# piotrkawa/audio-deepfake-adversarial-attacks

Measured on AMD Instinct MI355X. Metric: adversarial utterances/sec, PGD-40 LCNN+LFCC 4s@16kHz, higher is better.
Workload: dtype f32

## Files before the change

audio_deepfake_adversarial_attacks_amd/csrc/lfcc_stft.hip:

```cpp

#include <hip/hip_runtime.h>
#include <math.h>
#include <stdint.h>
#include <stdlib.h>

#include "advstep_frontend.h"
#include "advstep_common.h"

namespace {

constexpr int kN = 256;
constexpr int kNfft = 2 * kN;
constexpr int kBins = kN + 1;
constexpr int kWavesPerBlock = 4;
constexpr int kThreads = kWavesPerBlock * 64;
constexpr int kFramesPerBlockBwd = 4;

__device__ __forceinline__ float2 cmul(float2 a, float2 b) { return make_float2(a.x * b.x - a.y * b.y, a.x * b.y + a.y * b.x); }
__device__ __forceinline__ float2 cadd(float2 a, float2 b) { return make_float2(a.x + b.x, a.y + b.y); }
__device__ __forceinline__ float2 csub(float2 a, float2 b) { return make_float2(a.x - b.x, a.y - b.y); }
__device__ __forceinline__ float2 conjf2(float2 a) { return make_float2(a.x, -a.y); }

__device__ __forceinline__ void wave_lds_sync() {
    __builtin_amdgcn_fence(__ATOMIC_RELEASE, "workgroup");
    __builtin_amdgcn_wave_barrier();
    __builtin_amdgcn_fence(__ATOMIC_ACQUIRE, "workgroup");
}

#include "stft_tables.inc"

__device__ __forceinline__ float2 cmulf(float2 a, float2 b) {
    return make_float2(fmaf(a.x, b.x, -(a.y * b.y)), fmaf(a.x, b.y, a.y * b.x));
}
__device__ __forceinline__ float2 cmulc(float2 a, float cr, float ci) { return cmulf(a, make_float2(cr, ci)); }

template <bool INV>
__device__ __forceinline__ void fft4(float2 &a, float2 &b, float2 &c, float2 &d) {
    const float2 s02 = cadd(a, c), d02 = csub(a, c), s13 = cadd(b, d), d13 = csub(b, d);
    const float2 r = INV ? make_float2(-d13.y, d13.x) : make_float2(d13.y, -d13.x);
    a = cadd(s02, s13);
    b = cadd(d02, r);
    c = csub(s02, s13);
    d = csub(d02, r);
}

template <bool INV>
__device__ __forceinline__ void fft16(float2 (&x)[16]) {
    constexpr float C1 = 0.92387953251128674f, S1 = 0.38268343236508977f, H = 0.70710678118654752f;
#pragma unroll
    for (int n2 = 0; n2 < 4; ++n2) fft4<INV>(x[n2], x[4 + n2], x[8 + n2], x[12 + n2]);
    const float sg = INV ? 1.0f : -1.0f;
    x[4 + 1] = cmulc(x[4 + 1], C1, sg * S1);
    x[8 + 1] = cmulc(x[8 + 1], H, sg * H);
    x[12 + 1] = cmulc(x[12 + 1], S1, sg * C1);
    x[4 + 2] = cmulc(x[4 + 2], H, sg * H);
    x[8 + 2] = INV ? make_float2(-x[8 + 2].y, x[8 + 2].x) : make_float2(x[8 + 2].y, -x[8 + 2].x);
    x[12 + 2] = cmulc(x[12 + 2], -H, sg * H);
    x[4 + 3] = cmulc(x[4 + 3], S1, sg * C1);
    x[8 + 3] = cmulc(x[8 + 3], -H, sg * H);
    x[12 + 3] = cmulc(x[12 + 3], -C1, -sg * S1);
#pragma unroll
    for (int k1 = 0; k1 < 4; ++k1) fft4<INV>(x[4 * k1], x[4 * k1 + 1], x[4 * k1 + 2], x[4 * k1 + 3]);
#pragma unroll
    for (int i = 0; i < 4; ++i)
#pragma unroll
        for (int j = i + 1; j < 4; ++j) {
            const float2 t = x[4 * i + j];
            x[4 * i + j] = x[4 * j + i];
            x[4 * j + i] = t;
        }
}

__device__ __forceinline__ int here(int v) {
    asm volatile("" : "+v"(v));
    return v;
}

__device__ __forceinline__ void phase_done(float2 (&x)[16]) {
    asm volatile("" : "+v"(x[0].x), "+v"(x[0].y), "+v"(x[1].x), "+v"(x[1].y), "+v"(x[2].x), "+v"(x[2].y), "+v"(x[3].x), "+v"(x[3].y),
                      "+v"(x[4].x), "+v"(x[4].y), "+v"(x[5].x), "+v"(x[5].y), "+v"(x[6].x), "+v"(x[6].y), "+v"(x[7].x), "+v"(x[7].y)
                 :: "memory");
    asm volatile("" : "+v"(x[8].x), "+v"(x[8].y), "+v"(x[9].x), "+v"(x[9].y), "+v"(x[10].x), "+v"(x[10].y), "+v"(x[11].x), "+v"(x[11].y),
                      "+v"(x[12].x), "+v"(x[12].y), "+v"(x[13].x), "+v"(x[13].y), "+v"(x[14].x), "+v"(x[14].y), "+v"(x[15].x), "+v"(x[15].y)
                 :: "memory");
}

template <int BASE>
__device__ __forceinline__ void half_done(float2 (&x)[16]) {
    asm volatile("" : "+v"(x[BASE].x), "+v"(x[BASE].y), "+v"(x[BASE + 1].x), "+v"(x[BASE + 1].y), "+v"(x[BASE + 2].x), "+v"(x[BASE + 2].y),
                      "+v"(x[BASE + 3].x), "+v"(x[BASE + 3].y), "+v"(x[BASE + 4].x), "+v"(x[BASE + 4].y), "+v"(x[BASE + 5].x),
                      "+v"(x[BASE + 5].y), "+v"(x[BASE + 6].x), "+v"(x[BASE + 6].y), "+v"(x[BASE + 7].x), "+v"(x[BASE + 7].y)
                 :: "memory");
}

constexpr int kPitch = 17;
constexpr int kFrameSlots = 16 * kPitch;
constexpr int kGroup = 4;

__device__ __forceinline__ void lds_wave_fence() { asm volatile("s_waitcnt lgkmcnt(0)" ::: "memory"); }

template <bool INV>
__device__ __forceinline__ void fft256_reg(float2 (&x)[16], const float2 *twl, float2 *blk, int l) {
    fft16<INV>(x);
    phase_done(x);
#pragma unroll
    for (int j = 1; j < 16; ++j) {
        const float2 t = twl[l * kPitch + j];
        x[j] = cmulf(x[j], INV ? conjf2(t) : t);
    }
    lds_wave_fence();
#pragma unroll
    for (int j = 0; j < 16; ++j) blk[j * kPitch + l] = x[j];
    lds_wave_fence();
#pragma unroll
    for (int j = 0; j < 16; ++j) x[j] = blk[l * kPitch + j];
    fft16<INV>(x);
}

__device__ __forceinline__ int P(int i) { return i ^ (((i >> 4) & 3) * 5); }
constexpr int kNPad = kN + kN / 16;
constexpr int kStageTw = 3 * (4 + 16 + 64);

template <bool INV>
__device__ __forceinline__ void fft256(float2 *a, float2 *b, const float2 *__restrict__ tw, int lane) {
#pragma unroll
    for (int stage = 0; stage < 4; ++stage) {
        const int Ns = 1 << (2 * stage);
        const int k = lane & (Ns - 1);
        float2 v0 = a[P(lane)], v1 = a[P(lane + 64)], v2 = a[P(lane + 128)], v3 = a[P(lane + 192)];
        if (stage > 0) {
            const float2 *ts = tw + (stage == 1 ? 0 : (stage == 2 ? 12 : 60));
            float2 w1 = ts[k], w2 = ts[Ns + k], w3 = ts[2 * Ns + k];
            if (INV) w1 = conjf2(w1), w2 = conjf2(w2), w3 = conjf2(w3);
            v1 = cmul(v1, w1), v2 = cmul(v2, w2), v3 = cmul(v3, w3);
        }
        const float2 s02 = cadd(v0, v2), d02 = csub(v0, v2), s13 = cadd(v1, v3), d13 = csub(v1, v3);
        const float2 r = INV ? make_float2(-d13.y, d13.x) : make_float2(d13.y, -d13.x);
        const int j0 = ((lane - k) << 2) + k;
        b[P(j0)] = cadd(s02, s13);
        b[P(j0 + Ns)] = cadd(d02, r);
        b[P(j0 + 2 * Ns)] = csub(s02, s13);
        b[P(j0 + 3 * Ns)] = csub(d02, r);
        wave_lds_sync();
        float2 *t = a;
        a = b;
        b = t;
    }
}

__device__ __forceinline__ void load_frame(const float *__restrict__ xb, const float *__restrict__ w, int T, int f,
                                           int hop, float2 *z, int lane) {
    const int q_first = f * hop - kN;
    if (q_first >= 0 && q_first + kNfft <= T && ((q_first & 1) == 0) && ((reinterpret_cast<uintptr_t>(xb) & 7u) == 0)) {
        const float2 *x2 = reinterpret_cast<const float2 *>(xb + q_first);
        const float2 *w2 = reinterpret_cast<const float2 *>(w);
#pragma unroll
        for (int i = 0; i < 4; ++i) {
            const int n = lane + 64 * i;
            const float2 xv = x2[n], wv = w2[n];
            z[P(n)] = make_float2(wv.x * xv.x, wv.y * xv.y);
        }
        return;
    }
#pragma unroll
    for (int i = 0; i < 4; ++i) {
        const int n = lane + 64 * i;
        int q0 = f * hop + 2 * n - kN, q1 = q0 + 1;
        q0 = q0 < 0 ? -q0 : q0;
        q0 = q0 >= T ? 2 * (T - 1) - q0 : q0;
        q1 = q1 < 0 ? -q1 : q1;
        q1 = q1 >= T ? 2 * (T - 1) - q1 : q1;
        z[P(n)] = make_float2(w[2 * n] * xb[q0], w[2 * n + 1] * xb[q1]);
    }
}

__device__ __forceinline__ void unpack_real(const float2 *Z, const float2 *__restrict__ tw512, float2 *xs, int lane) {
    for (int k = lane; k < kN; k += 64) {
        const float2 zk = Z[P(k)], zc = conjf2(Z[P((kN - k) & (kN - 1))]);
        const float2 e = make_float2(0.5f * (zk.x + zc.x), 0.5f * (zk.y + zc.y));
        const float2 d = make_float2(0.5f * (zk.x - zc.x), 0.5f * (zk.y - zc.y));
        const float2 o = cmul(tw512[k], make_float2(d.y, -d.x));
        xs[k] = cadd(e, o);
    }
    if (lane == 0) xs[kN] = make_float2(Z[P(0)].x - Z[P(0)].y, 0.0f);
}

struct Lds {
    float2 a[kWavesPerBlock][kNPad];
    float2 b[kWavesPerBlock][kNPad];
    __device__ __forceinline__ float2 *xs_of(int wave) { return b[wave]; }
    __device__ __forceinline__ const float2 *xs_of(int wave) const { return b[wave]; }
    float2 tw[kStageTw];
    float2 tw512[kN];
    float red[kWavesPerBlock];
};

__device__ __forceinline__ float2 stage_twiddle(int m) {
    const int stage = m < 12 ? 1 : (m < 60 ? 2 : 3), base = stage == 1 ? 0 : (stage == 2 ? 12 : 60), Ns = 1 << (2 * stage);
    const int t = (m - base) / Ns + 1, k = (m - base) % Ns;
    return kTw256[(t * k * (64 / Ns)) & 255];
}

__device__ __forceinline__ void fill_twiddles(Lds &L) {
    for (int m = threadIdx.x; m < kN; m += kThreads) {
        if (m < kStageTw) L.tw[m] = stage_twiddle(m);
        L.tw512[m] = kTw512[m];
    }
}

constexpr int kFramesPerBlockFwd = 16;

__global__ __launch_bounds__(kThreads) void stft_bands_kernel(const float *__restrict__ x, const float *__restrict__ w,
                                                              const int32_t *__restrict__ fb_start,
                                                              const float *__restrict__ fb_w, int span,
                                                              float *__restrict__ band_db, float *__restrict__ bmax, int T,
                                                              int NF, int hop, int M) {
    __shared__ Lds L;
    fill_twiddles(L);
    __syncthreads();
    const int wave = threadIdx.x >> 6, lane = threadIdx.x & 63;
    const int64_t b = blockIdx.y;
    float vmax = -INFINITY;
    for (int r = 0; r < kFramesPerBlockFwd / kWavesPerBlock; ++r) {
        const int f = blockIdx.x * kFramesPerBlockFwd + r * kWavesPerBlock + wave;
        if (f >= NF) break;
        load_frame(x + b * T, w, T, f, hop, L.a[wave], lane);
        wave_lds_sync();
        fft256<false>(L.a[wave], L.b[wave], L.tw, lane);
        unpack_real(L.a[wave], L.tw512, L.xs_of(wave), lane);
        wave_lds_sync();
        float *row = band_db + (b * NF + f) * M;
        for (int m = lane; m < M; m += 64) {
            const int f0 = fb_start[m];
            float band = 0.0f;
            for (int j = 0; j < span; ++j) {
                const int k = f0 + j;
                if (k < kBins) {
                    const float2 z = L.xs_of(wave)[k];
                    band = fmaf(fb_w[m * span + j], fmaf(z.x, z.x, z.y * z.y), band);
                }
            }
            const float db = 3.010299956639812f * __log2f(band > kAmin ? band : (band != band ? band : kAmin));
            row[m] = db;
            vmax = max_nan(vmax, db);
        }
        wave_lds_sync();
    }
    vmax = wave_reduce(vmax, MaxNanOp());
    if (lane == 0) L.red[wave] = vmax;
    __syncthreads();
    if (threadIdx.x == 0) {
        float r = L.red[0];
        for (int i = 1; i < kWavesPerBlock; ++i) r = max_nan(r, L.red[i]);
        bmax[b * gridDim.x + blockIdx.x] = r;
    }
}

constexpr int kMaxSpanT = 8, kMaxBands = 128;

__device__ __forceinline__ void frame_spectrum(const float *__restrict__ xb, const float *__restrict__ w, int T, int f,
                                               int hop, Lds &L, int wave, int lane) {
    load_frame(xb, w, T, f, hop, L.a[wave], lane);
    wave_lds_sync();
    fft256<false>(L.a[wave], L.b[wave], L.tw, lane);
    unpack_real(L.a[wave], L.tw512, L.xs_of(wave), lane);
    wave_lds_sync();
}

__device__ __forceinline__ float2 one_sided_scale(float2 gk, int k) {
    if (k == 0 || k == kN) gk.y = 0.0f;
    else gk.x *= 0.5f, gk.y *= 0.5f;
    return gk;
}

template <bool PRESCALED>
__device__ __forceinline__ void spectrum_grad_to_frame(Lds &L, int wave, int lane, const float *__restrict__ w, float *dst,
                                                       bool live) {
    if (!PRESCALED) {
        for (int k = lane; k < kBins; k += 64) L.xs_of(wave)[k] = one_sided_scale(L.xs_of(wave)[k], k);
        wave_lds_sync();
    }
    for (int k = lane; k < kN; k += 64) {
        const float2 gk = L.xs_of(wave)[k], gc = conjf2(L.xs_of(wave)[kN - k]);
        const float2 e = cadd(gk, gc), d = csub(gk, gc);
        const float2 wd = cmul(conjf2(L.tw512[k]), d);
        L.a[wave][P(k)] = make_float2(e.x - wd.y, e.y + wd.x);
    }
    wave_lds_sync();
    fft256<true>(L.a[wave], L.b[wave], L.tw, lane);
    for (int n = lane; n < kN; n += 64) {
        const float2 z = L.a[wave][P(n)];
        const float2 wv = reinterpret_cast<const float2 *>(w)[n];
        reinterpret_cast<float2 *>(dst)[n] = live ? make_float2(wv.x * z.x, wv.y * z.y) : make_float2(0.0f, 0.0f);
    }
    wave_lds_sync();
}

template <int STRIDE>
__device__ __attribute__((noinline)) void overlap_add_frames_cold(const float *dframe, float *__restrict__ dxb, int f_base, int NF, int hop,
                                                                  int T, int tid, int nthreads);

template <int STRIDE>
__device__ __forceinline__ void overlap_add_frames(const float *dframe, float *__restrict__ dxb, int f_base, int NF, int hop, int T,
                                                   int tid, int nthreads) {
    const int p_lo = f_base * hop;
    const int frames_here = (NF - f_base) < kFramesPerBlockBwd ? (NF - f_base) : kFramesPerBlockBwd;
    const int p_hi = p_lo + (frames_here - 1) * hop + kNfft;
    auto add_from = [&](int p, float &acc) {
        if (p < p_lo || p >= p_hi) return;
#pragma unroll
        for (int fl = 0; fl < kFramesPerBlockBwd; ++fl) {
            const int n = p - p_lo - fl * hop;
            if (fl < frames_here && n >= 0 && n < kNfft) acc += dframe[fl * STRIDE + n];
        }
    };
    const bool near_left = p_lo < 2 * kN, near_right = p_hi > T;
    const int t_first = p_lo - kN, span_all = p_hi - p_lo;
    for (int i = tid; i < span_all; i += nthreads) {
        const int t = t_first + i;
        if (t < 0 || t >= T) continue;
        float acc = 0.0f;
        add_from(t + kN, acc);
        if (near_left && t >= 1 && t <= kN) add_from(kN - t, acc);
        if (near_right && t <= T - 2 && t >= T - 1 - kN) add_from(2 * (T - 1) - t + kN, acc);
        if (acc != 0.0f) atomicAdd(dxb + t, acc);
    }
    if (!(near_left || near_right)) return;
    for (int i = tid; i < span_all; i += nthreads) {
        const int p = p_lo + i, q = p - kN;
        int t = -1;
        if (q < 0) t = -q;
        else if (q >= T) t = 2 * (T - 1) - q;
        if (t < 0 || t >= T) continue;
        const int pd = t + kN;
        if (pd >= p_lo && pd < p_hi) continue;
        float acc = 0.0f;
        add_from(p, acc);
        if (acc != 0.0f) atomicAdd(dxb + t, acc);
    }
}

__device__ __forceinline__ void overlap_add_block(const float (*dframe)[kNfft], float *__restrict__ dxb, int f_base, int NF,
                                                  int hop, int T) {
    overlap_add_frames<kNfft>(&dframe[0][0], dxb, f_base, NF, hop, T, threadIdx.x, kThreads);
}

template <int STRIDE>
__device__ __attribute__((noinline)) void overlap_add_frames_cold(const float *dframe, float *__restrict__ dxb, int f_base, int NF, int hop,
                                                                  int T, int tid, int nthreads) {
    overlap_add_frames<STRIDE>(dframe, dxb, f_base, NF, hop, T, tid, nthreads);
}

template <int SPAN_CAP>
struct LdsBwd {
    Lds c;
    float dframe[kFramesPerBlockBwd][kNfft];
    float fbt_w[kBins * SPAN_CAP];
    int32_t fbt_start[kBins];
    float drow[kWavesPerBlock][kMaxBands];
};

template <int SPAN_CAP>
__global__ __launch_bounds__(kThreads) void stft_bands_backward_kernel(const float *__restrict__ x,
                                                                       const float *__restrict__ w,
                                                                       const float *__restrict__ dband,
                                                                       const int32_t *__restrict__ fbt_start,
                                                                       const float *__restrict__ fbt_w, int span_t,
                                                                       float *__restrict__ dx, int T, int NF, int hop,
                                                                       int M) {
    extern __shared__ __attribute__((aligned(16))) unsigned char raw[];
    LdsBwd<SPAN_CAP> &S = *reinterpret_cast<LdsBwd<SPAN_CAP> *>(raw);
    Lds &L = S.c;
    {
        static_assert(kN == kThreads, "one twiddle pair per thread");
        constexpr int kWIt = (kBins * SPAN_CAP + kThreads - 1) / kThreads;
        const int m = threadIdx.x, nw = kBins * span_t;
        const float2 t0 = stage_twiddle(m < kStageTw ? m : 0), t1 = kTw512[m];
        const int32_t s0 = fbt_start[m], s1 = fbt_start[kThreads + (m < kBins - kThreads ? m : 0)];
        float wq[kWIt];
#pragma unroll
        for (int j = 0; j < kWIt; ++j) {
            const int i = m + j * kThreads;
            wq[j] = fbt_w[i < nw ? i : nw - 1];
        }
        if (m < kStageTw) L.tw[m] = t0;
        L.tw512[m] = t1;
        S.fbt_start[m] = s0;
        if (m < kBins - kThreads) S.fbt_start[kThreads + m] = s1;
#pragma unroll
        for (int j = 0; j < kWIt; ++j) {
            const int i = m + j * kThreads;
            if (i < nw) S.fbt_w[i] = wq[j];
        }
    }
    __syncthreads();
    const int wave = threadIdx.x >> 6, lane = threadIdx.x & 63;
    const int64_t b = blockIdx.y;
    const int f_base = blockIdx.x * kFramesPerBlockBwd;
    const float *xb = x + b * T;
    for (int r = 0; r < kFramesPerBlockBwd / kWavesPerBlock; ++r) {
        const int fl = r * kWavesPerBlock + wave;
        const int f = f_base + fl;
        const bool live = f < NF;
        const float *drow_g = dband + (b * NF + (live ? f : NF - 1)) * M;
        for (int m = lane; m < M; m += 64) S.drow[wave][m] = drow_g[m];
        load_frame(xb, w, T, live ? f : NF - 1, hop, L.a[wave], lane);
        wave_lds_sync();
        fft256<false>(L.a[wave], L.b[wave], L.tw, lane);
        const float *drow = S.drow[wave];
        auto grad_of_bin = [&](int k, float2 xk) {
            const int m0 = S.fbt_start[k];
            float dp = 0.0f;
            for (int j = 0; j < span_t; ++j) {
                const int m = m0 + j;
                if (m < M) dp = fmaf(S.fbt_w[k * span_t + j], drow[m], dp);
            }
            return one_sided_scale(make_float2(2.0f * xk.x * dp, 2.0f * xk.y * dp), k);
        };
        {
            const float2 *Z = L.a[wave];
            for (int k = lane; k < kN; k += 64) {
                const float2 zk = Z[P(k)], zc = conjf2(Z[P((kN - k) & (kN - 1))]);
                const float2 e = make_float2(0.5f * (zk.x + zc.x), 0.5f * (zk.y + zc.y));
                const float2 d = make_float2(0.5f * (zk.x - zc.x), 0.5f * (zk.y - zc.y));
                const float2 o = cmul(L.tw512[k], make_float2(d.y, -d.x));
                L.xs_of(wave)[k] = grad_of_bin(k, cadd(e, o));
            }
            if (lane == 0) L.xs_of(wave)[kN] = grad_of_bin(kN, make_float2(Z[P(0)].x - Z[P(0)].y, 0.0f));
        }
        wave_lds_sync();
        spectrum_grad_to_frame<true>(L, wave, lane, w, S.dframe[fl], live);
    }
    __syncthreads();
    overlap_add_block(S.dframe, dx + b * T, f_base, NF, hop, T);
}

#ifndef STFT_FWD_GROUPS
#define STFT_FWD_GROUPS 2
#endif
constexpr int kGroupsPerWave = STFT_FWD_GROUPS;
constexpr int kBandsFramesPerBlock = kWavesPerBlock * kGroupsPerWave * kGroup;

struct LdsReg {
    float2 blk[kWavesPerBlock][kGroup][kFrameSlots];
    float2 twl[16 * kPitch];
    float red[kWavesPerBlock];
};

__device__ __forceinline__ void fill_reg_tables(LdsReg &S) {
    for (int m = threadIdx.x; m < kN; m += kThreads) S.twl[(m >> 4) * kPitch + (m & 15)] = kTw256[((m >> 4) * (m & 15)) & 255];
}

__device__ __forceinline__ void load_frame_reg(const float *__restrict__ xb, const float2 *__restrict__ win2, int T, int f, int hop,
                                               float2 (&x)[16], int l) {
    const int q_first = f * hop - kN;
    if (q_first >= 0 && q_first + kNfft <= T && ((q_first & 1) == 0) && ((reinterpret_cast<uintptr_t>(xb) & 7u) == 0)) {
        const float2 *x2 = reinterpret_cast<const float2 *>(xb + q_first);
        float2 v[16];
#pragma unroll
        for (int r = 0; r < 16; ++r) v[r] = x2[16 * r + l];
#pragma unroll
        for (int r = 0; r < 16; ++r) {
            const float2 wv = win2[16 * r + l];
            x[r] = make_float2(wv.x * v[r].x, wv.y * v[r].y);
        }
        return;
    }
#pragma unroll
    for (int r = 0; r < 16; ++r) {
        const int n = 16 * r + l;
        int q0 = q_first + 2 * n, q1 = q0 + 1;
        q0 = q0 < 0 ? -q0 : q0;
        q0 = q0 >= T ? 2 * (T - 1) - q0 : q0;
        q1 = q1 < 0 ? -q1 : q1;
        q1 = q1 >= T ? 2 * (T - 1) - q1 : q1;
        const float2 wv = win2[n];
        x[r] = make_float2(wv.x * xb[q0], wv.y * xb[q1]);
    }
}

__device__ __forceinline__ void park_vector(float2 *blk, const float2 (&x)[16], int l) {
#pragma unroll
    for (int r = 0; r < 16; ++r) blk[r * kPitch + l] = x[r];
    if (l == 0) {
#pragma unroll
        for (int r = 0; r < 16; ++r) blk[((r + 15) & 15) * kPitch + 16] = x[r];
    }
}
__device__ __forceinline__ float2 mirror_of(const float2 *blk, int r, int l) { return blk[(15 - r) * kPitch + (16 - l)]; }

__device__ __forceinline__ void unpack_real_reg(float2 (&x)[16], float &nyq, float2 *blk, int l) {
    lds_wave_fence();
    park_vector(blk, x, l);
    lds_wave_fence();
    nyq = 2.0f * (x[0].x - x[0].y);
    const int lt = here(l);
#pragma unroll
    for (int r = 0; r < 16; ++r) {
        if (r == 8) half_done<0>(x);
        const float2 zc = conjf2(mirror_of(blk, r, l));
        const float2 e = cadd(x[r], zc), d = csub(x[r], zc);
        x[r] = cadd(e, cmulf(kTw512[lt + 16 * r], make_float2(d.y, -d.x)));
    }
}

constexpr int kRegSpan = 4;

struct LdsRegFwd {
    LdsReg c;
    float fbw[kMaxBands * kRegSpan];
    int32_t fbs[kMaxBands];
};

__global__ __launch_bounds__(kThreads) void stft_bands_reg_kernel(const float *__restrict__ x, const float *__restrict__ w,
                                                                  const int32_t *__restrict__ fb_start,
                                                                  const float *__restrict__ fb_w, int span,
                                                                  float *__restrict__ band_db, float *__restrict__ bmax, int T,
                                                                  int NF, int hop, int M, int bmax_tail) {
    __shared__ LdsRegFwd SF;
    LdsReg &S = SF.c;
    fill_reg_tables(S);
    for (int i = threadIdx.x; i < kMaxBands * kRegSpan; i += kThreads) {
        const int m = i / kRegSpan, j = i % kRegSpan;
        SF.fbw[i] = (m < M && j < span) ? 0.25f * fb_w[m * span + j] : 0.0f;
    }
    for (int m = threadIdx.x; m < kMaxBands; m += kThreads) SF.fbs[m] = m < M ? fb_start[m] : 0;
    const int wave = threadIdx.x >> 6, lane = threadIdx.x & 63, fs = lane >> 4, l = lane & 15;
    __syncthreads();
    const int64_t b = blockIdx.y;
    float2 *blk = S.blk[wave][fs];
    float vmax = -INFINITY;
    for (int g = 0; g < kGroupsPerWave; ++g) {
        const int f0 = blockIdx.x * kBandsFramesPerBlock + (wave * kGroupsPerWave + g) * kGroup;
        if (f0 >= NF) break;
        const int f = f0 + fs;
        const bool live = f < NF;
        float2 xr[16];
        load_frame_reg(x + b * T, reinterpret_cast<const float2 *>(w), T, live ? f : NF - 1, hop, xr, here(l));
        fft256_reg<false>(xr, S.twl, blk, l);
        float nyq;
        unpack_real_reg(xr, nyq, blk, l);
        phase_done(xr);
        float *pw = reinterpret_cast<float *>(blk);
        lds_wave_fence();
#pragma unroll
        for (int r = 0; r < 16; ++r) pw[l + 16 * r] = fmaf(xr[r].x, xr[r].x, xr[r].y * xr[r].y);
        if (l == 0) pw[kN] = nyq * nyq;
        if (l >= 1 && l <= kRegSpan) pw[kN + l] = 0.0f;
        lds_wave_fence();
        float *row = band_db + (b * NF + (live ? f : NF - 1)) * M;
#pragma unroll
        for (int half = 0; half < 2; ++half) {
            int k0[4];
            float wt[4][kRegSpan], pv[4][kRegSpan];
#pragma unroll
            for (int i = 0; i < 4; ++i) k0[i] = SF.fbs[l + 16 * (4 * half + i)];
#pragma unroll
            for (int i = 0; i < 4; ++i)
#pragma unroll
                for (int j = 0; j < kRegSpan; ++j) {
                    wt[i][j] = SF.fbw[(l + 16 * (4 * half + i)) * kRegSpan + j];
                    pv[i][j] = pw[k0[i] + j];
                }
#pragma unroll
            for (int i = 0; i < 4; ++i) {
                const int m = l + 16 * (4 * half + i);
                float band = 0.0f;
#pragma unroll
                for (int j = 0; j < kRegSpan; ++j) band = fmaf(wt[i][j], pv[i][j], band);
                const float db = 3.010299956639812f * __log2f(band > kAmin ? band : (band != band ? band : kAmin));
                if (live && m < M) {
                    row[m] = db;
                    vmax = max_nan(vmax, db);
                }
            }
        }
        lds_wave_fence();
    }
    vmax = wave_reduce(vmax, MaxNanOp());
    if (lane == 0) S.red[wave] = vmax;
    __syncthreads();
    if (threadIdx.x == 0) {
        float r = S.red[0];
        for (int i = 1; i < kWavesPerBlock; ++i) r = max_nan(r, S.red[i]);
        bmax[b * gridDim.x + blockIdx.x] = r;
        const int total = gridDim.x * gridDim.y;
        for (int j = (int)b * gridDim.x + blockIdx.x; j < bmax_tail; j += total) bmax[total + j] = -INFINITY;
    }
}

template <int STRIDE>
__device__ __forceinline__ void overlap_add_interior(const float *df, float *__restrict__ out, int lane, float (&carry)[6],
                                                     bool carry_in, bool carry_out) {
    constexpr int HOP = 160, kSpan = 3 * HOP + kNfft, kShared = kNfft - HOP;
    static_assert(4 * HOP == 640 && kSpan <= 16 * 64, "slices");
#pragma unroll
    for (int j = 0; j < 16; ++j) {
        if (j % 4 == 0) lds_wave_fence();
        float acc = 0.0f;
#pragma unroll
        for (int fl = 0; fl < 4; ++fl) {
            const int lo = HOP * fl - 64 * j, hi = lo + kNfft;
            if (hi <= 0 || lo >= 64) continue;
            if (lo <= 0 && hi >= 64) {
                acc += df[fl * STRIDE + lane - lo];
            } else {
                const int n = lane - lo;
                if ((unsigned)n < (unsigned)kNfft) acc += df[fl * STRIDE + n];
            }
        }
        const int i = lane + 64 * j;
        if (j < 6) {
            const bool shared = i < kShared;
            if (carry_in) {
                out[i] = shared ? acc + carry[j] : acc;
            } else if (j < 5) {
                atomicAdd(out + i, acc);
            } else {
                if (shared) atomicAdd(out + i, acc);
                else out[i] = acc;
            }
        } else if (j < 10) {
            out[i] = acc;
        } else {
            if (carry_out) carry[j - 10] = acc;
            else if (i < kSpan) atomicAdd(out + i, acc);
        }
    }
}

template <int SPAN_CAP>
struct LdsRegBwd {
    LdsReg c;
    float fbt_w[(kBins + 1) * SPAN_CAP];
    int32_t fbt_start[kBins + 1];
};

#ifndef STFT_BWD_GROUPS
#define STFT_BWD_GROUPS 4
#endif
constexpr int kBwdGroupsPerWave = STFT_BWD_GROUPS;
constexpr int kBwdFramesPerBlock = kWavesPerBlock * kBwdGroupsPerWave * kGroup;

#ifndef STFT_BWD_WAVES
#define STFT_BWD_WAVES 4
#endif
template <int SPAN_CAP>
__global__ __launch_bounds__(kThreads) __attribute__((amdgpu_waves_per_eu(STFT_BWD_WAVES, STFT_BWD_WAVES)))
void stft_bands_backward_reg_kernel(const float *__restrict__ x,
                                                                           const float *__restrict__ w,
                                                                           const float *__restrict__ dband,
                                                                           const int32_t *__restrict__ fbt_start,
                                                                           const float *__restrict__ fbt_w, int span_t,
                                                                           float *__restrict__ dx, int T, int NF, int hop,
                                                                           int M, const float *__restrict__ band_db,
                                                                           const float *__restrict__ stats) {
    extern __shared__ __attribute__((aligned(16))) unsigned char raw[];
    LdsRegBwd<SPAN_CAP> &S = *reinterpret_cast<LdsRegBwd<SPAN_CAP> *>(raw);
    float fix_share = 0.0f, fix_max = 0.0f;
    bool fix = false;
    if (stats != nullptr) {
        const float s2 = stats[2];
        if (s2 != 0.0f) {
            fix = true;
            fix_max = stats[0];
            fix_share = s2 / (stats[1] > 0.0f ? stats[1] : 1.0f);
        }
    }
    fill_reg_tables(S.c);
    for (int i = threadIdx.x; i < kBins * SPAN_CAP; i += kThreads) {
        const int k = i / SPAN_CAP, j = i % SPAN_CAP;
        S.fbt_w[i] = j < span_t ? fbt_w[k * span_t + j] : 0.0f;
    }
    for (int i = threadIdx.x; i < kBins; i += kThreads) S.fbt_start[i] = fbt_start[i];
    const int wave = threadIdx.x >> 6, lane = threadIdx.x & 63, fs = lane >> 4, l = lane & 15;
    __syncthreads();
    const int64_t b = blockIdx.y;
    const float *xb = x + b * T;
    float2 *blk = S.c.blk[wave][fs];
    float carry[6] = {0.0f, 0.0f, 0.0f, 0.0f, 0.0f, 0.0f};
    bool carried = false;
    auto interior = [&](int g0) {
        return hop == 160 && g0 + kGroup <= NF && g0 * hop >= 2 * kN && g0 * hop + 3 * hop + kNfft <= T;
    };
    for (int g = 0; g < kBwdGroupsPerWave; ++g) {
        const int f0 = blockIdx.x * kBwdFramesPerBlock + (wave * kBwdGroupsPerWave + g) * kGroup;
        if (f0 >= NF) break;
        const int f = f0 + fs;
        const bool live = f < NF;
        const int fc = live ? f : NF - 1;
        float dreg[kMaxBands / 16];
        {
            const float *src = dband + (b * NF + fc) * M;
#pragma unroll
            for (int i = 0; i < kMaxBands / 16; ++i) {
                const int m = l + 16 * i;
                dreg[i] = m < M ? src[m] : 0.0f;
            }
            if (fix) {
                const float *dbrow = band_db + (b * NF + fc) * M;
#pragma unroll
                for (int i = 0; i < kMaxBands / 16; ++i) {
                    const int m = l + 16 * i;
                    const float db = m < M ? dbrow[m] : 0.0f;
                    if (m < M && db == fix_max) dreg[i] += fix_share * dlog_of_db(db);
                }
            }
        }
        float2 xr[16];
        load_frame_reg(xb, reinterpret_cast<const float2 *>(w), T, fc, hop, xr, here(l));
        phase_done(xr);
        fft256_reg<false>(xr, S.c.twl, blk, l);
        float nyq;
        unpack_real_reg(xr, nyq, blk, l);
        phase_done(xr);
        float *drow = reinterpret_cast<float *>(blk);
        lds_wave_fence();
#pragma unroll
        for (int i = 0; i < kMaxBands / 16; ++i) drow[l + 16 * i] = dreg[i];
        if (l < SPAN_CAP) drow[kMaxBands + l] = 0.0f;
#pragma unroll
        for (int q = 0; q < 4; ++q) {
            lds_wave_fence();
            int m0[4];
#pragma unroll
            for (int i = 0; i < 4; ++i) m0[i] = S.fbt_start[l + 16 * (4 * q + i)];
#pragma unroll
            for (int i = 0; i < 4; ++i) {
                const int r = 4 * q + i;
                float dp = 0.0f;
#pragma unroll
                for (int j = 0; j < SPAN_CAP; ++j) dp = fmaf(S.fbt_w[(l + 16 * r) * SPAN_CAP + j], drow[m0[i] + j], dp);
                const bool dc = r == 0 && l == 0;
                const float c = dc ? dp : 0.5f * dp;
                xr[r] = make_float2(c * xr[r].x, dc ? 0.0f : c * xr[r].y);
            }
            asm volatile("" : "+v"(xr[4 * q].x), "+v"(xr[4 * q].y), "+v"(xr[4 * q + 1].x), "+v"(xr[4 * q + 1].y), "+v"(xr[4 * q + 2].x),
                              "+v"(xr[4 * q + 2].y), "+v"(xr[4 * q + 3].x), "+v"(xr[4 * q + 3].y) :: "memory");
        }
        float g_nyq = 0.0f;
        if (l == 0) {
            const int m0n = S.fbt_start[kN];
            float dpn = 0.0f;
#pragma unroll
            for (int j = 0; j < SPAN_CAP; ++j) dpn = fmaf(S.fbt_w[kN * SPAN_CAP + j], drow[m0n + j], dpn);
            g_nyq = dpn * nyq;
        }
        phase_done(xr);
        lds_wave_fence();
        park_vector(blk, xr, l);
        lds_wave_fence();
        int lp = here(l);
#pragma unroll
        for (int r = 0; r < 16; ++r) {
            if (r == 8) half_done<0>(xr);
            float2 gc = conjf2(mirror_of(blk, r, l));
            if (r == 0 && l == 0) gc = make_float2(g_nyq, 0.0f);
            const float2 e = cadd(xr[r], gc), d = csub(xr[r], gc);
            const float2 wd = cmulf(conjf2(kTw512[lp + 16 * r]), d);
            xr[r] = make_float2(e.x - wd.y, e.y + wd.x);
        }
        fft256_reg<true>(xr, S.c.twl, blk, l);
        lds_wave_fence();
        lp = here(l);
#pragma unroll
        for (int r = 0; r < 16; ++r) {
            const float2 wv = reinterpret_cast<const float2 *>(w)[lp + 16 * r];
            blk[l + 16 * r] = live ? make_float2(wv.x * xr[r].x, wv.y * xr[r].y) : make_float2(0.0f, 0.0f);
        }
        lds_wave_fence();
        const float *df = reinterpret_cast<const float *>(S.c.blk[wave][0]);
        if (interior(f0)) {
            const bool carry_out = g + 1 < kBwdGroupsPerWave && f0 + kGroup < NF && interior(f0 + kGroup);
            overlap_add_interior<2 * kFrameSlots>(df, dx + b * T + (f0 * hop - kN), lane, carry, carried, carry_out);
            carried = carry_out;
        } else {
            overlap_add_frames_cold<2 * kFrameSlots>(df, dx + b * T, f0, NF, hop, T, lane, 64);
            carried = false;
        }
        lds_wave_fence();
    }
}

constexpr int kMelMax = 80;
constexpr int kMelMaxSpan = 48;

struct LdsMel {
    Lds c;
    float2 y[kWavesPerBlock][kMelMax];
    float stage[2][kMelMax][kFramesPerBlockFwd + 1];
};

template <int CAP>
struct MelTaps {
    float w[2][CAP];
    int f0[2];
};

template <int CAP>
__device__ __forceinline__ void load_mel_taps(MelTaps<CAP> &t, int lane, const int32_t *__restrict__ fb_start,
                                              const float *__restrict__ fb_w, int span, int M) {
#pragma unroll
    for (int pass = 0; pass < 2; ++pass) {
        const int m = lane + 64 * pass;
        const bool live = m < M;
        const int f0 = live ? fb_start[m] : 0;
        t.f0[pass] = f0;
#pragma unroll
        for (int j = 0; j < CAP; ++j) t.w[pass][j] = (live && j < span && f0 + j < kBins) ? fb_w[m * span + j] : 0.0f;
    }
}

template <int CAP>
__device__ __forceinline__ void mel_bands(const Lds &L, int wave, int lane, const MelTaps<CAP> &t, int M, float2 *y) {
#pragma unroll
    for (int pass = 0; pass < 2; ++pass) {
        const int m = lane + 64 * pass;
        if (m < M) {
            float re = 0.0f, im = 0.0f;
#pragma unroll
            for (int j = 0; j < CAP; ++j) {
                const int k = t.f0[pass] + j < kBins ? t.f0[pass] + j : kBins - 1;
                const float2 z = L.xs_of(wave)[k];
                re = fmaf(t.w[pass][j], z.x, re);
                im = fmaf(t.w[pass][j], z.y, im);
            }
            y[m] = make_float2(re, im);
        }
    }
}

template <int CAP>
__global__ __launch_bounds__(kThreads) void stft_mel_kernel(const float *__restrict__ x, const float *__restrict__ w,
                                                            const int32_t *__restrict__ fb_start,
                                                            const float *__restrict__ fb_w, int span,
                                                            float *__restrict__ out, int T, int NF, int hop, int M) {
    extern __shared__ __attribute__((aligned(16))) unsigned char raw[];
    LdsMel &S = *reinterpret_cast<LdsMel *>(raw);
    Lds &L = S.c;
    fill_twiddles(L);
    __syncthreads();
    const int wave = threadIdx.x >> 6, lane = threadIdx.x & 63;
    const int64_t b = blockIdx.y;
    const int f_base = blockIdx.x * kFramesPerBlockFwd;
    MelTaps<CAP> taps;
    load_mel_taps(taps, lane, fb_start, fb_w, span, M);
    for (int r = 0; r < kFramesPerBlockFwd / kWavesPerBlock; ++r) {
        const int fl = r * kWavesPerBlock + wave, f = f_base + fl;
        if (f >= NF) break;
        frame_spectrum(x + b * T, w, T, f, hop, L, wave, lane);
        mel_bands(L, wave, lane, taps, M, S.y[wave]);
        wave_lds_sync();
        for (int m = lane; m < M; m += 64) {
            const float2 v = S.y[wave][m];
            S.stage[0][m][fl] = sqrtf(v.x * v.x + v.y * v.y);
            S.stage[1][m][fl] = atan2f(v.y, v.x);
        }
        wave_lds_sync();
    }
    __syncthreads();
    const int frames_here = (NF - f_base) < kFramesPerBlockFwd ? (NF - f_base) : kFramesPerBlockFwd;
    for (int i = threadIdx.x; i < 2 * M * kFramesPerBlockFwd; i += kThreads) {
        const int fl = i % kFramesPerBlockFwd, row = i / kFramesPerBlockFwd, plane = row / M, m = row - plane * M;
        if (fl < frames_here) out[((b * 2 + plane) * M + m) * NF + f_base + fl] = S.stage[plane][m][fl];
    }
}

struct LdsMelBwd {
    Lds c;
    float dframe[kFramesPerBlockBwd][kNfft];
    float2 y[kWavesPerBlock][kMelMax];
    float stage[2][kMelMax][kFramesPerBlockBwd + 1];
};

template <int CAP, int SPT>
__global__ __launch_bounds__(kThreads) void stft_mel_backward_kernel(const float *__restrict__ x, const float *__restrict__ w,
                                                                     const float *__restrict__ dout,
                                                                     const int32_t *__restrict__ fb_start,
                                                                     const float *__restrict__ fb_w, int span,
                                                                     const int32_t *__restrict__ fbt_start,
                                                                     const float *__restrict__ fbt_w, int span_t,
                                                                     float *__restrict__ dx, int T, int NF, int hop, int M) {
    extern __shared__ __attribute__((aligned(16))) unsigned char raw[];
    LdsMelBwd &S = *reinterpret_cast<LdsMelBwd *>(raw);
    Lds &L = S.c;
    fill_twiddles(L);
    const int wave = threadIdx.x >> 6, lane = threadIdx.x & 63;
    const int64_t b = blockIdx.y;
    const int f_base = blockIdx.x * kFramesPerBlockBwd;
    const int frames_here = (NF - f_base) < kFramesPerBlockBwd ? (NF - f_base) : kFramesPerBlockBwd;
    for (int i = threadIdx.x; i < 2 * M * kFramesPerBlockBwd; i += kThreads) {
        const int fl = i % kFramesPerBlockBwd, row = i / kFramesPerBlockBwd, plane = row / M, m = row - plane * M;
        S.stage[plane][m][fl] = fl < frames_here ? dout[((b * 2 + plane) * M + m) * NF + f_base + fl] : 0.0f;
    }
    __syncthreads();
    const float *xb = x + b * T;
    MelTaps<CAP> taps;
    load_mel_taps(taps, lane, fb_start, fb_w, span, M);
    constexpr int kBinPasses = (kBins + 63) / 64;
    float tw_t[kBinPasses][SPT];
    int m0_t[kBinPasses];
#pragma unroll
    for (int p = 0; p < kBinPasses; ++p) {
        const int k = lane + 64 * p;
        const bool in = k < kBins;
        m0_t[p] = in ? fbt_start[k] : 0;
#pragma unroll
        for (int j = 0; j < SPT; ++j) tw_t[p][j] = (in && j < span_t && m0_t[p] + j < M) ? fbt_w[k * span_t + j] : 0.0f;
    }
    for (int r = 0; r < kFramesPerBlockBwd / kWavesPerBlock; ++r) {
        const int fl = r * kWavesPerBlock + wave, f = f_base + fl;
        const bool live = f < NF;
        frame_spectrum(xb, w, T, live ? f : NF - 1, hop, L, wave, lane);
        mel_bands(L, wave, lane, taps, M, S.y[wave]);
        wave_lds_sync();
        for (int m = lane; m < M; m += 64) {
            const float2 v = S.y[wave][m];
            const float gm = S.stage[0][m][fl], gp = S.stage[1][m][fl];
            const float n2 = v.x * v.x + v.y * v.y;
            float2 gy = make_float2(0.0f, 0.0f);
            if (n2 > 0.0f) {
                const float inv = 1.0f / sqrtf(n2), inv2 = 1.0f / n2;
                gy.x = gm * v.x * inv - gp * v.y * inv2;
                gy.y = gm * v.y * inv + gp * v.x * inv2;
            }
            S.y[wave][m] = gy;
        }
        wave_lds_sync();
#pragma unroll
        for (int p = 0; p < kBinPasses; ++p) {
            const int k = lane + 64 * p;
            if (k < kBins) {
                float re = 0.0f, im = 0.0f;
#pragma unroll
                for (int j = 0; j < SPT; ++j) {
                    const int m = m0_t[p] + j < M ? m0_t[p] + j : M - 1;
                    const float2 gy = S.y[wave][m];
                    re = fmaf(tw_t[p][j], gy.x, re);
                    im = fmaf(tw_t[p][j], gy.y, im);
                }
                L.xs_of(wave)[k] = make_float2(re, im);
            }
        }
        wave_lds_sync();
        spectrum_grad_to_frame<false>(L, wave, lane, w, S.dframe[fl], live);
    }
    __syncthreads();
    overlap_add_block(S.dframe, dx + b * T, f_base, NF, hop, T);
}

struct LdsMelBwdOut {
    Lds c;
    float dframe[kFramesPerBlockBwd][kNfft];
    float2 y[kWavesPerBlock][kMelMax];
    float stage[4][kMelMax][kFramesPerBlockBwd + 1];
};

template <int SPT>
__global__ __launch_bounds__(kThreads) void stft_mel_backward_out_kernel(const float *__restrict__ w, const float *__restrict__ dout,
                                                                         const float *__restrict__ out,
                                                                         const int32_t *__restrict__ fbt_start,
                                                                         const float *__restrict__ fbt_w, int span_t,
                                                                         float *__restrict__ dx, int T, int NF, int hop, int M) {
    extern __shared__ __attribute__((aligned(16))) unsigned char raw[];
    LdsMelBwdOut &S = *reinterpret_cast<LdsMelBwdOut *>(raw);
    Lds &L = S.c;
    fill_twiddles(L);
    const int wave = threadIdx.x >> 6, lane = threadIdx.x & 63;
    const int64_t b = blockIdx.y;
    const int f_base = blockIdx.x * kFramesPerBlockBwd;
    const int frames_here = (NF - f_base) < kFramesPerBlockBwd ? (NF - f_base) : kFramesPerBlockBwd;
    for (int i = threadIdx.x; i < 4 * M * kFramesPerBlockBwd; i += kThreads) {
        const int fl = i % kFramesPerBlockBwd, row = i / kFramesPerBlockBwd, plane = row / M, m = row - plane * M;
        const float *src = plane < 2 ? dout : out;
        S.stage[plane][m][fl] = fl < frames_here ? src[((b * 2 + (plane & 1)) * M + m) * NF + f_base + fl] : 0.0f;
    }
    constexpr int kBinPasses = (kBins + 63) / 64;
    float tw_t[kBinPasses][SPT];
    int m0_t[kBinPasses];
#pragma unroll
    for (int p = 0; p < kBinPasses; ++p) {
        const int k = lane + 64 * p;
        const bool in = k < kBins;
        m0_t[p] = in ? fbt_start[k] : 0;
#pragma unroll
        for (int j = 0; j < SPT; ++j) tw_t[p][j] = (in && j < span_t && m0_t[p] + j < M) ? fbt_w[k * span_t + j] : 0.0f;
    }
    __syncthreads();
    for (int r = 0; r < kFramesPerBlockBwd / kWavesPerBlock; ++r) {
        const int fl = r * kWavesPerBlock + wave;
        const bool live = f_base + fl < NF;
        for (int m = lane; m < M; m += 64) {
            const float gm = S.stage[0][m][fl], gp = S.stage[1][m][fl], mag = S.stage[2][m][fl], ph = S.stage[3][m][fl];
            float2 gy = make_float2(0.0f, 0.0f);
            if (mag > 0.0f) {
                float sn, cs;
                sincosf(ph, &sn, &cs);
                const float q = gp / mag;
                gy.x = gm * cs - q * sn;
                gy.y = gm * sn + q * cs;
            }
            S.y[wave][m] = gy;
        }
        wave_lds_sync();
#pragma unroll
        for (int p = 0; p < kBinPasses; ++p) {
            const int k = lane + 64 * p;
            if (k < kBins) {
                float re = 0.0f, im = 0.0f;
#pragma unroll
                for (int j = 0; j < SPT; ++j) {
                    const int m = m0_t[p] + j < M ? m0_t[p] + j : M - 1;
                    const float2 gy = S.y[wave][m];
                    re = fmaf(tw_t[p][j], gy.x, re);
                    im = fmaf(tw_t[p][j], gy.y, im);
                }
                L.xs_of(wave)[k] = make_float2(re, im);
            }
        }
        wave_lds_sync();
        spectrum_grad_to_frame<false>(L, wave, lane, w, S.dframe[fl], live);
    }
    __syncthreads();
    overlap_add_block(S.dframe, dx + b * T, f_base, NF, hop, T);
}

constexpr int kMelRegSpan = 16;
constexpr int kMelBandsPerLane = (kMelMax + 15) / 16;

struct LdsMelReg {
    LdsReg c;
    float fbw[kMelMax * kMelRegSpan];
    int32_t fbs[kMelMax];
};
static_assert(2 * kMelMax * (kBandsFramesPerBlock + 1) * sizeof(float) <= sizeof(LdsReg::blk), "the output tile aliases the exchange blocks");

__global__ __launch_bounds__(kThreads) void stft_mel_reg_kernel(const float *__restrict__ x, const float *__restrict__ w,
                                                                const int32_t *__restrict__ fb_start,
                                                                const float *__restrict__ fb_w, int span,
                                                                float *__restrict__ out, int T, int NF, int hop, int M) {
    extern __shared__ __attribute__((aligned(16))) unsigned char raw[];
    LdsMelReg &SF = *reinterpret_cast<LdsMelReg *>(raw);
    LdsReg &S = SF.c;
    fill_reg_tables(S);
    for (int i = threadIdx.x; i < kMelMax * kMelRegSpan; i += kThreads) {
        const int m = i / kMelRegSpan, j = i % kMelRegSpan;
        SF.fbw[i] = (m < M && j < span) ? 0.5f * fb_w[m * span + j] : 0.0f;
    }
    for (int m = threadIdx.x; m < kMelMax; m += kThreads) {
        const int k0 = m < M ? fb_start[m] : 0;
        SF.fbs[m] = k0 + kMelRegSpan <= kBins + 15 ? k0 : kBins + 15 - kMelRegSpan;
    }
    const int wave = threadIdx.x >> 6, lane = threadIdx.x & 63, fs = lane >> 4, l = lane & 15;
    __syncthreads();
    const int64_t b = blockIdx.y;
    const int f_base = blockIdx.x * kBandsFramesPerBlock;
    float2 *blk = S.blk[wave][fs];
    float mag[kGroupsPerWave][kMelBandsPerLane], ph[kGroupsPerWave][kMelBandsPerLane];
#pragma unroll
    for (int g = 0; g < kGroupsPerWave; ++g) {
        const int f0 = f_base + (wave * kGroupsPerWave + g) * kGroup;
#pragma unroll
        for (int i = 0; i < kMelBandsPerLane; ++i) mag[g][i] = ph[g][i] = 0.0f;
        if (f0 >= NF) continue;
        const int f = f0 + fs;
        const bool live = f < NF;
        float2 xr[16];
        load_frame_reg(x + b * T, reinterpret_cast<const float2 *>(w), T, live ? f : NF - 1, hop, xr, here(l));
        phase_done(xr);
        fft256_reg<false>(xr, S.twl, blk, l);
        float nyq;
        unpack_real_reg(xr, nyq, blk, l);
// ... 364 lines not shown
```

Baseline: 2029.

## Software-pipeline twiddle, window and frame loads in LFCC STFT backward kernel

Restructures the backward STFT-bands kernel so that global and LDS loads for twiddles, window coefficients and frame samples are issued ahead of use and waited on with explicit partial s_waitcnt values. The FFT helper gains an optional twiddle-preload path and a prefetch callback that fires between the LDS transpose store and load. The real-unpack steps now consume mirror values in batches of four. This is meant to hide memory latency behind FFT arithmetic, at the cost of more live registers (possible occupancy loss) and hand-coded waitcnt encodings that must stay correct.

```diff
diff --git a/audio_deepfake_adversarial_attacks_amd/csrc/lfcc_stft.hip b/audio_deepfake_adversarial_attacks_amd/csrc/lfcc_stft.hip
--- a/audio_deepfake_adversarial_attacks_amd/csrc/lfcc_stft.hip
+++ b/audio_deepfake_adversarial_attacks_amd/csrc/lfcc_stft.hip
@@ -99,18 +99,32 @@
 
 __device__ __forceinline__ void lds_wave_fence() { asm volatile("s_waitcnt lgkmcnt(0)" ::: "memory"); }
 
-template <bool INV>
-__device__ __forceinline__ void fft256_reg(float2 (&x)[16], const float2 *twl, float2 *blk, int l) {
+__device__ __forceinline__ void lds_batch_arrived() { __builtin_amdgcn_s_waitcnt(0xc07f); }
+__device__ __forceinline__ void global_batch_arrived() { __builtin_amdgcn_s_waitcnt(0x0f70); }
+
+struct NoPrefetch {
+    __device__ __forceinline__ void operator()() const {}
+};
+
+template <bool INV, bool AHEAD = false, class Prefetch = NoPrefetch>
+__device__ __forceinline__ void fft256_reg(float2 (&x)[16], const float2 *twl, float2 *blk, int l, Prefetch &&prefetch = Prefetch()) {
+    float2 t[16];
+    if (AHEAD) {
+#pragma unroll
+        for (int j = 1; j < 16; ++j) t[j] = twl[l * kPitch + j];
+    }
     fft16<INV>(x);
     phase_done(x);
+    if (AHEAD) lds_batch_arrived();
 #pragma unroll
     for (int j = 1; j < 16; ++j) {
-        const float2 t = twl[l * kPitch + j];
-        x[j] = cmulf(x[j], INV ? conjf2(t) : t);
+        const float2 tj = AHEAD ? t[j] : twl[l * kPitch + j];
+        x[j] = cmulf(x[j], INV ? conjf2(tj) : tj);
     }
     lds_wave_fence();
 #pragma unroll
     for (int j = 0; j < 16; ++j) blk[j * kPitch + l] = x[j];
+    prefetch();
     lds_wave_fence();
 #pragma unroll
     for (int j = 0; j < 16; ++j) x[j] = blk[l * kPitch + j];
@@ -479,6 +493,42 @@
     }
 }
 
+__device__ __forceinline__ void request_frame_reg(const float *__restrict__ xb, int T, int f, int hop, float2 (&v)[16], int l) {
+    const int q_first = f * hop - kN;
+    if (q_first >= 0 && q_first + kNfft <= T && ((q_first & 1) == 0) && ((reinterpret_cast<uintptr_t>(xb) & 7u) == 0)) {
+        const float2 *x2 = reinterpret_cast<const float2 *>(xb + q_first);
+#pragma unroll
+        for (int r = 0; r < 16; ++r) v[r] = x2[16 * r + l];
+        return;
+    }
+#pragma unroll
+    for (int r = 0; r < 16; ++r) {
+        const int n = 16 * r + l;
+        int q0 = q_first + 2 * n, q1 = q0 + 1;
+        q0 = q0 < 0 ? -q0 : q0;
+        q0 = q0 >= T ? 2 * (T - 1) - q0 : q0;
+        q1 = q1 < 0 ? -q1 : q1;
+        q1 = q1 >= T ? 2 * (T - 1) - q1 : q1;
+        v[r] = make_float2(xb[q0], xb[q1]);
+        if (r % 4 == 3)
+            asm volatile("" : "+v"(v[r - 3].x), "+v"(v[r - 3].y), "+v"(v[r - 2].x), "+v"(v[r - 2].y), "+v"(v[r - 1].x), "+v"(v[r - 1].y),
+                              "+v"(v[r].x), "+v"(v[r].y) :: "memory");
+    }
+}
+__device__ __forceinline__ void request_window_reg(const float2 *__restrict__ win2, float2 (&wv)[16], int lw) {
+#pragma unroll
+    for (int r = 0; r < 16; ++r) wv[r] = win2[16 * r + lw];
+}
+__device__ __forceinline__ void window_frame_reg(const float2 (&v)[16], const float2 (&wv)[16], float2 (&x)[16]) {
+#pragma unroll
+    for (int r = 0; r < 16; ++r) x[r] = make_float2(wv[r].x * v[r].x, wv[r].y * v[r].y);
+}
+template <int LO, int HI>
+__device__ __forceinline__ void request_tw512_reg(float2 (&tw)[16], int lt) {
+#pragma unroll
+    for (int r = LO; r < HI; ++r) tw[r] = kTw512[lt + 16 * r];
+}
+
 __device__ __forceinline__ void park_vector(float2 *blk, const float2 (&x)[16], int l) {
 #pragma unroll
     for (int r = 0; r < 16; ++r) blk[r * kPitch + l] = x[r];
@@ -501,6 +551,30 @@
         const float2 zc = conjf2(mirror_of(blk, r, l));
         const float2 e = cadd(x[r], zc), d = csub(x[r], zc);
         x[r] = cadd(e, cmulf(kTw512[lt + 16 * r], make_float2(d.y, -d.x)));
+    }
+}
+
+constexpr int kMirrorBatch = 4;
+__device__ __forceinline__ void unpack_real_reg_rolling(float2 (&x)[16], float &nyq, float2 *blk, int l, float2 (&tw)[16], int lt) {
+    lds_wave_fence();
+    park_vector(blk, x, l);
+    lds_wave_fence();
+    nyq = 2.0f * (x[0].x - x[0].y);
+#pragma unroll
+    for (int h = 0; h < 16 / kMirrorBatch; ++h) {
+        if (h == 0) request_tw512_reg<8, 12>(tw, lt);
+        if (h == 1) request_tw512_reg<12, 16>(tw, lt);
+        float2 zc[kMirrorBatch];
+#pragma unroll
+        for (int i = 0; i < kMirrorBatch; ++i) zc[i] = conjf2(mirror_of(blk, kMirrorBatch * h + i, l));
+        lds_batch_arrived();
+#pragma unroll
+        for (int i = 0; i < kMirrorBatch; ++i) {
+            const int r = kMirrorBatch * h + i;
+            const float2 e = cadd(x[r], zc[i]), d = csub(x[r], zc[i]);
+            x[r] = cadd(e, cmulf(tw[r], make_float2(d.y, -d.x)));
+        }
+        if (h == 1) half_done<0>(x);
     }
 }
 
@@ -683,6 +757,7 @@
     auto interior = [&](int g0) {
         return hop == 160 && g0 + kGroup <= NF && g0 * hop >= 2 * kN && g0 * hop + 3 * hop + kNfft <= T;
     };
+    const float2 *win2 = reinterpret_cast<const float2 *>(w);
     for (int g = 0; g < kBwdGroupsPerWave; ++g) {
         const int f0 = blockIdx.x * kBwdFramesPerBlock + (wave * kBwdGroupsPerWave + g) * kGroup;
         if (f0 >= NF) break;
@@ -707,12 +782,16 @@
                 }
             }
         }
-        float2 xr[16];
-        load_frame_reg(xb, reinterpret_cast<const float2 *>(w), T, fc, hop, xr, here(l));
+        float2 xv[16], wv[16];
+        request_frame_reg(xb, T, fc, hop, xv, l);
+        request_window_reg(win2, wv, here(l));
+        float2 xr[16], tw[16];
+        window_frame_reg(xv, wv, xr);
         phase_done(xr);
-        fft256_reg<false>(xr, S.c.twl, blk, l);
+        int lt = l;
+        fft256_reg<false, true>(xr, S.c.twl, blk, l, [&] { lt = here(l); request_tw512_reg<0, 8>(tw, lt); });
         float nyq;
-        unpack_real_reg(xr, nyq, blk, l);
+        unpack_real_reg_rolling(xr, nyq, blk, l, tw, lt);
         phase_done(xr);
         float *drow = reinterpret_cast<float *>(blk);
         lds_wave_fence();
@@ -721,6 +800,10 @@
         if (l < SPAN_CAP) drow[kMaxBands + l] = 0.0f;
 #pragma unroll
         for (int q = 0; q < 4; ++q) {
+            if (q == 3) {
+                lt = here(l);
+                request_tw512_reg<0, 8>(tw, lt);
+            }
             lds_wave_fence();
             int m0[4];
 #pragma unroll
@@ -750,24 +833,30 @@
         lds_wave_fence();
         park_vector(blk, xr, l);
         lds_wave_fence();
-        int lp = here(l);
-#pragma unroll
-        for (int r = 0; r < 16; ++r) {
-            if (r == 8) half_done<0>(xr);
-            float2 gc = conjf2(mirror_of(blk, r, l));
-            if (r == 0 && l == 0) gc = make_float2(g_nyq, 0.0f);
-            const float2 e = cadd(xr[r], gc), d = csub(xr[r], gc);
-            const float2 wd = cmulf(conjf2(kTw512[lp + 16 * r]), d);
-            xr[r] = make_float2(e.x - wd.y, e.y + wd.x);
-        }
-        fft256_reg<true>(xr, S.c.twl, blk, l);
-        lds_wave_fence();
-        lp = here(l);
-#pragma unroll
-        for (int r = 0; r < 16; ++r) {
-            const float2 wv = reinterpret_cast<const float2 *>(w)[lp + 16 * r];
-            blk[l + 16 * r] = live ? make_float2(wv.x * xr[r].x, wv.y * xr[r].y) : make_float2(0.0f, 0.0f);
-        }
+#pragma unroll
+        for (int h = 0; h < 16 / kMirrorBatch; ++h) {
+            if (h == 0) request_tw512_reg<8, 12>(tw, lt);
+            if (h == 1) request_tw512_reg<12, 16>(tw, lt);
+            float2 gc[kMirrorBatch];
+#pragma unroll
+            for (int i = 0; i < kMirrorBatch; ++i) gc[i] = conjf2(mirror_of(blk, kMirrorBatch * h + i, l));
+            lds_batch_arrived();
+            if (h == 0 && l == 0) gc[0] = make_float2(g_nyq, 0.0f);
+#pragma unroll
+            for (int i = 0; i < kMirrorBatch; ++i) {
+                const int r = kMirrorBatch * h + i;
+                const float2 e = cadd(xr[r], gc[i]), d = csub(xr[r], gc[i]);
+                const float2 wd = cmulf(conjf2(tw[r]), d);
+                xr[r] = make_float2(e.x - wd.y, e.y + wd.x);
+            }
+            if (h == 1) half_done<0>(xr);
+        }
+        fft256_reg<true, true>(xr, S.c.twl, blk, l, [&] { request_window_reg(win2, wv, here(l)); });
+        lds_wave_fence();
+        global_batch_arrived();
+#pragma unroll
+        for (int r = 0; r < 16; ++r)
+            blk[l + 16 * r] = live ? make_float2(wv[r].x * xr[r].x, wv[r].y * xr[r].y) : make_float2(0.0f, 0.0f);
         lds_wave_fence();
         const float *df = reinterpret_cast<const float *>(S.c.blk[wave][0]);
         if (interior(f0)) {
```

Result: no change. 2037, median of 6 (+0.4%).
